# PraKesEy/EEGNetReplication

Hardware: AMD Instinct MI355X
Metric: train trials/sec (fwd+bwd) EEGNet-8,2 22ch x 256 (higher is better)
Workload: dtype fp32; 1 GPU; EEGNet-8,2 train step (fwd+CE+bwd+clamps+Adam), 22ch x 256, batch 4096/GPU, p=0.5, fp32 HIP kernels; model=EEGNet-8,2, global_batch=4096, seq_len=256, channels=22, parallelism=dp1

## Files before the change

eegnetreplication_amd/csrc/eegnet_stream.hip:

```cpp

namespace eeg {

constexpr int NTB = 512;
constexpr int NWB = NTB / 64;
constexpr int RPW = F2MAX / NWB;
constexpr int WGPC = 2;
constexpr int WPEB = NWB * WGPC / 4;

__device__ __forceinline__ int fir_row(int lane) { return (lane >> 3) & 1; }
__device__ __forceinline__ int fir_oct(int lane) { return (lane & 7) | ((lane >> 4) << 3); }
#define EEG_XP(TT, g) (((TT) && ((TT) & 3) == 0) ? (TT) : (g).XP)
#define EEG_NO(TT) ((TT) ? ((TT) + 7) / 8 : ((T + 7) >> 3))
#define EEG_MO(TT) ((TT) ? (((TT) + 7) / 8 + 31) / 32 : 4)

typedef __attribute__((address_space(1))) void gvoid_t;
typedef __attribute__((address_space(3))) void lvoid_t;
__device__ __forceinline__ void x_dma(const float* __restrict__ xb, int C, int T, int RS, int LP, float* Xs,
                                      int wave, int lane) {
    if ((T & 255) == 0) {
        const int np = T >> 8;
        for (int i = wave; i < C * np; i += NWB) {
            const int c = i / np, p = i - c * np;
            __builtin_amdgcn_global_load_lds((gvoid_t*)(xb + (size_t)c * T + 256 * p + 4 * lane),
                                             (lvoid_t*)(Xs + c * RS + LP + 256 * p), 16, 0, 0);
// ... 577 lines not shown
            float a[4];
#pragma unroll
            for (int i = 0; i < 4; ++i) a[i] = (4 * q + i < T) ? w[G_::OFF + i] : 0.f;
            s0 += (a[0] + a[1]) + (a[2] + a[3]);
#pragma unroll
            for (int d = 0; d < K1; ++d) {
                float acc = G0[d];
#pragma unroll
                for (int i = 0; i < 4; ++i) acc = fmaf(a[i], w[G_::OFF + i + d], acc);
                G0[d] = acc;
            }
        }
        float* orow = out + (size_t)b * NV;
#pragma unroll
        for (int i = 0; i < NEI; ++i) {
            if (ea[i] >= 0) {
                const float* xa = Xb + LP + ea[i];
                float acc = 0.f;
                if (eb[i] >= 0) {
                    const float* xb2 = Xb + LP + eb[i];
                    for (int c = 0; c < C; ++c) acc = fmaf(xa[c * RS], xb2[c * RS], acc);
                } else {
                    for (int c = 0; c < C; ++c) acc += xa[c * RS];
                }
                orow[K1 + 1 + tid + NTB * i] = acc;
            }
        }
        constexpr int NR = (K1 + 1 + 3) & ~3, NQ = NR / 4;
        float rv[NR];
#pragma unroll
        for (int d = 0; d < K1; ++d) rv[d] = G0[d];
        rv[K1] = s0;
#pragma unroll
        for (int i = K1 + 1; i < NR; ++i) rv[i] = 0.f;
        wave_reduce<NR>(rv);
        if ((lane & 15) == 0) {
            const int r0 = (lane >> 4) * NQ;
#pragma unroll
            for (int j = 0; j < NQ; ++j)
                if (j + r0 <= K1) red[wave * (K1 + 1) + j + r0] = rv[j];
        }
        __syncthreads();
        if (tid <= K1) {
            float t = 0.f;
            for (int w = 0; w < NWB; ++w) t += red[w * (K1 + 1) + tid];
            orow[tid] = t;
        }
    }
}

template <int K1, int CC, int TT, int FF, bool FOLD>
__device__ __forceinline__ void pass_b_body(const Geo& g, const float* __restrict__ prm,
                                            const float* coef,
                                            const float* __restrict__ vg,
                                            const uint8_t* __restrict__ mask2,
                                            float* __restrict__ d2g, float* __restrict__ E1g,
                                            float* __restrict__ E2g, float* __restrict__ q3g,
                                            float* __restrict__ r3g, float* __restrict__ part,
                                            FinArgs fa, const FoldCall& fc, float* sm) {
    EEG_DIMS_NT(g, NTB);
    TRACE(g, 1, TR_ENTRY);
    unsigned dk0;
    if (FOLD) {
        const eegnet_fold f = fold_rec(fc);
        char* ws = (char*)f.ws;
        prm = f.params;
        coef = (const float*)(ws + fc.off.coef);
        vg = (const float*)(ws + fc.off.v);
        mask2 = nullptr;
        d2g = (float*)(ws + fc.off.d2); E1g = (float*)(ws + fc.off.E1); E2g = (float*)(ws + fc.off.E2);
        q3g = (float*)(ws + fc.off.q3); r3g = (float*)(ws + fc.off.r3);
        part = (float*)(ws + fc.off.partB);
        fa = fold_fin(fc, f, TK_B, 1, 0, true, false, g.nparam);
        dk0 = fold_drop_key(fc, f, 0);
    } else {
        dk0 = drop_key(g, 0);
    }
    float* D2s = sm;
    float* Qs0 = D2s + F2 * RS2;
    float* Wt = Qs0 + 2 * F2 * RS2;
    const int tid = threadIdx.x, lane = tid & 63;
    const int wave = __builtin_amdgcn_readfirstlane(tid >> 6);
    int b0, b1;
    trial_range(g, b0, b1);
    const int NO = EEG_NO(TT);
    constexpr int MO = EEG_MO(TT);
    const int hr = fir_row(lane), oh = RPW * wave + hr;
    constexpr bool VPF = TT != 0;
    float vpf[MO][8];
    if (VPF && b0 < b1) v_load<MO>(vg, b0, F2, NO, oh, lane, vpf);

    for (int i = tid; i < 3 * F2 * RS2; i += NTB) sm[i] = 0.f;
    for (int i = tid; i < F2MAX * (K2 + F2MAX); i += NTB) {
        float v = 0.f;
        if (i < F2MAX * K2) { if (i < F2 * K2) v = prm[g.o_w2 + i]; }
        else {
            const int j = (i - F2MAX * K2) / F2MAX, c = (i - F2MAX * K2) % F2MAX;
            if (j < F2 && c < F2) v = prm[g.o_W3 + j * F2 + c];
        }
        Wt[i] = v;
    }
    float sr[RPW], sr2[RPW];
#pragma unroll
    for (int r = 0; r < RPW; ++r) { sr[r] = 0.f; sr2[r] = 0.f; }
    float alh, beh, gah, bth;
    {
        const int oo = oh < F2 ? oh : 0;
        alh = coef[CF_AL2 * CSTR + oo]; beh = coef[CF_BE2 * CSTR + oo];
        gah = prm[g.o_g2 + oo]; bth = prm[g.o_b2 + oo];
    }
    __syncthreads();

    TRACE(g, 1, TR_PRO);
    TRACE_DECL();
    drain_prologue_loads();
    for (int b = b0; b < b1; ++b) {
        const int bn = b + 1;
        pace_prio(b - b0, b1 - b0);
        float* Qs = Qs0 + ((b - b0) & 1) * F2 * RS2;
        float vc[MO][8];
        if constexpr (VPF) {
#pragma unroll
            for (int m = 0; m < MO; ++m)
#pragma unroll
                for (int i = 0; i < 8; ++i) vc[m][i] = vpf[m][i];
            if (bn < b1) v_load<MO>(vg, bn, F2, NO, oh, lane, vpf);
        } else {
            v_load<MO>(vg, b, F2, NO, oh, lane, vc);
        }
        TRACE_PH(g, 1, 0, tph_);
        float d2v[MO][2], e1v[MO][2], e2v[MO][2];
        if (oh < F2) {
            float* drow = D2s + oh * RS2 + LP2;
#pragma unroll
            for (int m = 0; m < MO; ++m) {
                const int oc = fir_oct(lane) + 32 * m;
                if (oc >= NO) break;
#pragma unroll
                for (int h = 0; h < 2; ++h) {
                    const int q = 2 * oc + h;
                    float pe = 0.f, e1 = 0.f, e2 = 0.f;
#pragma unroll
                    for (int i = 4 * h; i < 4 * h + 4; ++i) {
                        const float xh = fmaf(alh, vc[m][i], beh);
                        const float z = fmaf(gah, xh, bth);
                        const float dz = elu_d(z);
                        pe += z > 0.f ? z : dz - 1.f;
                        e1 += dz;
                        e2 = fmaf(dz, xh, e2);
                    }
                    const float d2 = q < T1 ? pe * 0.25f * keep_mul(g, mask2, dk0, (unsigned)((b * F2 + oh) * T1 + q)) : 0.f;
                    d2v[m][h] = d2; e1v[m][h] = e1; e2v[m][h] = e2;
                    if (q < T1) drow[q] = d2;
                }
            }
        }
        wave_lds_fence();
        TRACE_PH(g, 1, 1, tph_);
#pragma unroll
        for (int r = 0; r < RPW; ++r) {
            const int o = RPW * wave + r;
            if (o < F2) {
                const float* dr = D2s + o * RS2 + LP2 - 7;
                const float* w2 = Wt + o * K2;
                for (int t = lane; t < T1; t += 64) {
                    float a = 0.f;
#pragma unroll
                    for (int k = 0; k < K2; ++k) a = fmaf(w2[k], dr[t + k], a);
                    Qs[o * RS2 + t] = a;
                    q3g[((size_t)b * F2 + o) * T1 + t] = a;
                }
            }
        }
        TRACE_PH(g, 1, 2, tph_);
        if (oh < F2) {
#pragma unroll
            for (int m = 0; m < MO; ++m) {
                const int oc = fir_oct(lane) + 32 * m;
                if (oc >= NO) break;
#pragma unroll
                for (int h = 0; h < 2; ++h) {
                    const int q = 2 * oc + h;
                    if (q < T1) {
                        const size_t gi = ((size_t)b * F2 + oh) * T1 + q;
                        st_pol<EEGNET_NT_MID>(d2v[m][h], d2g + gi); st_pol<EEGNET_NT_MID>(e1v[m][h], E1g + gi);
                        st_pol<EEGNET_NT_MID>(e2v[m][h], E2g + gi);
                    }
                }
            }
        }
        TRACE_PH(g, 1, 3, tph_);
        barrier_lds();
        TRACE_PH(g, 1, 4, tph_);
        for (int t = lane; t < T1; t += 64) {
            float qv[F2MAX];
#pragma unroll
            for (int i = 0; i < F2MAX; ++i) qv[i] = i < F2 ? Qs[i * RS2 + t] : 0.f;
#pragma unroll
            for (int r = 0; r < RPW; ++r) {
                const int o = RPW * wave + r;
                if (o < F2) {
                    const float* w3 = Wt + F2MAX * K2 + o * F2MAX;
                    float rr = 0.f;
#pragma unroll
                    for (int i = 0; i < F2MAX; ++i) rr = fmaf(w3[i], qv[i], rr);
                    r3g[((size_t)b * F2 + o) * T1 + t] = rr;
                    sr[r] += rr;
                    sr2[r] = fmaf(rr, rr, sr2[r]);
                }
            }
        }
        TRACE_PH(g, 1, 5, tph_);
    }
    TRACE_LOOP(g, 1);
    tail_prio();
    {
        float rv[4] = {sr[0], sr[1], sr2[0], sr2[1]};
        wave_reduce<4>(rv);
        const int k = lane >> 4, o = RPW * wave + (k & 1);
        if ((lane & 15) == 0 && o < F2) {
            float* row = part + (size_t)blockIdx.x * g.nB;
            pub(row + ((k < 2 ? 0 : F2) + o), rv[0]);
        }
    }
    {
        double* dsm = (double*)sm;
        if (grid_reduce(g, part, g.nB, fa, dsm)) { fin2(g, dsm + 2, fa); TRACE(g, 1, TR_FIN); }
    }
}

template <int K1, int CC, int TT, int FF, bool FOLD = false>
__global__ __launch_bounds__(NTB, WPEB) void k_pass_b(Geo g, const float* __restrict__ prm,
                                                      const float* coef,
                                                      const float* __restrict__ vg,
                                                      const uint8_t* __restrict__ mask2,
                                                      float* __restrict__ d2g, float* __restrict__ E1g,
                                                      float* __restrict__ E2g, float* __restrict__ q3g,
                                                      float* __restrict__ r3g, float* __restrict__ part,
                                                      FinArgs fa, FoldCall fc) {
    extern __shared__ __attribute__((aligned(16))) float sm[];
    pass_b_body<K1, CC, TT, FF, FOLD>(g, prm, coef, vg, mask2, d2g, E1g, E2g, q3g, r3g, part, fa, fc, sm);
}

#ifndef EEGNET_LDSX_E
#define EEGNET_LDSX_E 0
#endif
template <int K1, int CC, int TT, int FF, bool FOLD>
__device__ __forceinline__ void pass_e_body(const Geo& g, const float* prm,
                                            const float* coef,
                                            const float* __restrict__ x,
                                            const float* __restrict__ sg, const float* __restrict__ vg,
                                            const float* __restrict__ dp2g,
                                            float* __restrict__ part, FinArgs fa, const FoldCall& fc, float* sm) {
    using G_ = KG<K1>;
    EEG_DIMS_NT(g, NTB);
    const int XP = EEG_XP(TT, g);
    TRACE(g, 4, TR_ENTRY);
    const int64_t* perm = nullptr;
    long long row0 = 0;
    if (FOLD) {
        const eegnet_fold f = fold_rec(fc);
        char* ws = (char*)f.ws;
        prm = f.params;
        coef = (const float*)(ws + fc.off.coef);
        x = f.x;
        perm = f.perm; row0 = fc.row0;
        sg = (const float*)(ws + fc.off.s);
        vg = (const float*)(ws + fc.off.v);
        dp2g = (const float*)(ws + fc.off.dp2);
        part = (float*)(ws + fc.off.partE);
        fa = fold_fin(fc, f, TK_E, 0, 0, false, true, g.nparam);
    }
    constexpr int NTS = FF ? 1 : RPW;
    const int D = FF ? 2 : g.D;
    const int QR = FF ? FF / 2 : g.QR;
    float* const Ss = sm;
    float* const Dys = Ss + F2 * RS;
    float* const Xb = Dys + F2 * RS;
    float* const DP = Xb + C * RS;
    float* red = sm;
    const int tid = threadIdx.x, lane = tid & 63;
    const int wave = __builtin_amdgcn_readfirstlane(tid >> 6);
    int b0, b1;
    trial_range(g, b0, b1);
    const int li = lane & 15, lk = lane >> 4;
    constexpr bool XDMA = TT != 0;
    static_assert(!XDMA || (CC && FF), "LDS-DMA staging is specialised to compile-time C and F2");

    TRACE_PS(g, 0);
    if constexpr (!XDMA) zero_fill<false>(sm, (2 * F2 + C) * RS, F2, RS, LP, T, tid);
    TRACE_PS(g, 1);
    float tap[NTS][K1];
    float* CT = DP + ((F2 * T1 + 3) & ~3);
    const int NO = EEG_NO(TT);
    constexpr int MO = EEG_MO(TT);
    const int hr = fir_row(lane), oh = RPW * wave + hr;
    constexpr bool ONEOC = FF && TT && (EEG_NO(TT) <= 32) && (FF == RPW * NWB);
    constexpr bool EINPL = ONEOC || XDMA;
    float* const Eb = EINPL ? Dys : Ss;
    constexpr bool XDMA_ = TT != 0;
    constexpr bool DPDMA_ = XDMA_ && FF && ((FF * (TT / 4)) % 256 == 0);
    constexpr bool PIPEE = ONEOC && XDMA_ && DPDMA_ && (TT / 4 == 64) && (TT == 256);
    float sdyl = 0.f, sdyvl = 0.f;
    constexpr int NWT = (15 + K1 - 1) / 16 + 1;
    floatx4 cq[RPW][NWT];
#pragma unroll
    for (int r = 0; r < RPW; ++r)
#pragma unroll
        for (int j = 0; j < NWT; ++j) cq[r][j] = (floatx4){0.f, 0.f, 0.f, 0.f};
    const int wpc = NWB / NCT;
    const bool gemm_on = wave < wpc * NCT;
    const int ct = gemm_on ? wave / wpc : 0, part_ = gemm_on ? wave - ct * wpc : 0;
    const int kg0 = (NT16 * part_) / wpc, kg1 = gemm_on ? (NT16 * (part_ + 1)) / wpc : 0;
    floatx4 xacc = {0.f, 0.f, 0.f, 0.f};
    constexpr int MS = TT ? (TT + 63) / 64 : 16;
    float pws[XDMA ? 1 : RPW][XDMA ? 1 : MS];
    auto s_rows_load = [&](int bb) {
        if constexpr (!XDMA) {
#pragma unroll
            for (int r = 0; r < RPW; ++r) {
                const float* src = sg + ((size_t)bb * F2 + min(RPW * wave + r, F2 - 1)) * s_pitch(T);
#pragma unroll
                for (int k = 0; k < MS; ++k) pws[r][k] = src[min(lane + 64 * k, T - 1)];
            }
        }
    };
    auto s_rows_put = [&]() {
        if constexpr (!XDMA) {
#pragma unroll
            for (int r = 0; r < RPW; ++r) {
                const int o = RPW * wave + r;
#pragma unroll
                for (int k = 0; k < MS; ++k)
                    if (o < F2 && lane + 64 * k < T) Ss[o * RS + LP + lane + 64 * k] = pws[r][k];
            }
        }
    };
    float pfx[XDMA ? 1 : PF];
    constexpr bool VPF = XDMA;
    float vpf[MO][8];
    constexpr int NDP = (CC && TT) ? (FF * (TT / 4) + NTB - 1) / NTB : 8;
    const int ndp = F2 * T1;
    float pdp[NDP];
    constexpr bool DPDMA = TT && FF && ((FF * (TT / 4)) % 256 == 0);
    if (b0 < b1) {
        if constexpr (XDMA) s_dma_asm(sg + (size_t)b0 * F2 * s_pitch(T), F2, T, RS, LP, Ss, wave, lane);
        else s_rows_load(b0);
        TRACE_PS(g, 3);
        if constexpr (DPDMA) flat_dma_asm(dp2g + (size_t)b0 * ndp, ndp, DP, wave, lane);
        else {
#pragma unroll
            for (int j = 0; j < NDP; ++j) pdp[j] = dp2g[(size_t)b0 * ndp + min(tid + NTB * j, ndp - 1)];
#pragma unroll
            for (int j = 0; j < NDP; ++j)
                if (tid + NTB * j < ndp) DP[tid + NTB * j] = pdp[j];
            for (int i = tid + NTB * NDP; i < ndp; i += NTB) DP[i] = dp2g[(size_t)b0 * ndp + i];
        }
        if constexpr (VPF) v_load<MO>(vg, b0, F2, NO, oh, lane, vpf);
        TRACE_PS(g, 4);
    }
    if constexpr (XDMA) zero_pads(sm, 2 * F2 + C, RS, LP, T, tid);
    load_taps<K1, NTS>(g, prm, D, F2, wave, tap);
    TRACE_PS(g, 2);
    {
        float cv = 0.f;
#pragma unroll
        for (int k = 0; k < 8 * RPW; ++k) {
            const int o = RPW * wave + (k >> 3), f = k & 7;
            if (o < F2 && f < 7) {
                const float* src = f == 0 ? coef + CF_AL2 * CSTR : f == 1 ? coef + CF_BE2 * CSTR
                                 : f == 2 ? prm + g.o_g2 : f == 3 ? prm + g.o_b2 : f == 4 ? coef + CF_AO * CSTR
                                 : f == 5 ? coef + CF_BO * CSTR : coef + CF_CO * CSTR;
                const float v = ldc(src + o);
                cv = lane == k ? v : cv;
            }
        }
        if (lane < 8 * RPW && RPW * wave + (lane >> 3) < F2) CT[8 * RPW * wave + lane] = cv;
    }
    adam_scalars_publish(g, fa);
    const int step0 = adam_step0(g, fa);
    if constexpr (XDMA) barrier_vm<0>();
    else __syncthreads();
    if constexpr (!XDMA) {
        if (b0 < b1) {
            s_rows_put();
            x_prefetch<PF, NTB>(x + fold_row(perm, row0, b0) * (C * XP), C, T, pfx, tid);
            x_store<PF, NTB>(pfx, C, T, RS, LP, Xb, tid);
        }
        __syncthreads();
    }

    TRACE(g, 4, TR_PRO);
    TRACE_DECL();
    drain_prologue_loads();
    for (int b = b0; b < b1; ++b) {
        const int bn = b + 1;
        pace_prio(b - b0, b1 - b0);
        float vc[MO][8];
        if constexpr (VPF) {
#pragma unroll
            for (int m = 0; m < MO; ++m)
#pragma unroll
                for (int i = 0; i < 8; ++i) vc[m][i] = vpf[m][i];
            if constexpr (PIPEE)
                if (bn < b1) v_load<MO>(vg, bn, F2, NO, oh, lane, vpf);
        } else {
            v_load<MO>(vg, b, F2, NO, oh, lane, vc);
        }
        TRACE_PH(g, 4, 0, tph_);
        if (oh < F2) {
            float* drow = Dys + oh * RS + LP;
            const floatx4 c0 = lds_ld4(CT + 8 * oh), c1 = lds_ld4(CT + 8 * oh + 4);
            const float alh = c0[0], beh = c0[1], gah = c0[2], bth = c0[3];
            const float Aoh = c1[0], Boh = c1[1], Coh = c1[2];
#pragma unroll
            for (int m = 0; m < MO; ++m) {
                const int oc = fir_oct(lane) + 32 * m;
                if (oc >= NO) break;
                float dpq[2];
#pragma unroll
                for (int h = 0; h < 2; ++h)
                    dpq[h] = EEGNET_LDSX_E == 1 ? 0.01f * (oc + h) : (2 * oc + h < T1) ? DP[oh * T1 + 2 * oc + h] * 0.25f : 0.f;
                float dy[8];
#pragma unroll
                for (int i = 0; i < 8; ++i) {
                    const bool in = 8 * oc + i < T;
                    const float v = in ? vc[m][i] : 0.f;
                    const float xh = fmaf(alh, v, beh);
                    const float z = fmaf(gah, xh, bth);
                    const float dz = dpq[i >> 2] * elu_d(z);
                    float d = fmaf(Aoh, dz, fmaf(Coh, xh, Boh));
                    d = in ? d : 0.f;
                    dy[i] = d;
                    sdyl += d;
                    sdyvl = fmaf(d, v, sdyvl);
                }
                if (EEGNET_LDSX_E != 5)
                    lds_st_oct(drow + 8 * oc, oc, (floatx4){dy[0], dy[1], dy[2], dy[3]}, (floatx4){dy[4], dy[5], dy[6], dy[7]});
            }
        }
        TRACE_PH(g, 4, 1, tph_);
        wave_lds_fence();
        if constexpr (PIPEE) {
            if (bn < b1) {
#pragma unroll
                for (int r = 0; r < RPW; ++r) {
                    const int o = RPW * wave + r;
                    if (EEGNET_LDSX_E != 7) dma4(dp2g + (size_t)bn * ndp + o * T1 + lane, DP + o * T1);
                }
            }
        }
        if constexpr (XDMA)
            if (EEGNET_LDSX_E != 7) x_dma_asm(x + fold_row(perm, row0, b) * (C * XP), C, T, XP, RS, LP, Xb, wave, lane);
        TRACE_PH(g, 4, 2, tph_);
        {
            float tl[K1];
            half_taps<K1, NTS>(tap, hr, tl);
            if constexpr (ONEOC) {
                constexpr int NT16C = (TT + 15) / 16, KQC = (NT16C + 3) / 4, NQ = RPW * KQC * NWT;
                const int oc = fir_oct(lane);
                float w[4 * G_::NW8];
                if (EEGNET_LDSX_E == 2) {
#pragma unroll
                    for (int i = 0; i < 4 * G_::NW8; ++i) w[i] = 0.001f * (lane + i);
                } else
                    lds_window<G_::NW8>(Dys + oh * RS + 8 * oc, w);
                float e[8];
#pragma unroll
                for (int i = 0; i < 8; ++i) e[i] = 0.f;
#pragma unroll
                for (int m = 0; m < K1; ++m) {
#pragma unroll
                    for (int i = 0; i < 8; ++i) e[i] = fmaf(tl[K1 - 1 - m], w[G_::OFFD + i + m], e[i]);
#pragma unroll
                    for (int n = (m * NQ) / K1; n < ((m + 1) * NQ) / K1; ++n) {
                        const int r = n / (KQC * NWT), ks = (n / NWT) % KQC, j = n % NWT;
                        const int o = RPW * wave + r, a = 4 * ks + lk;
                        const bool on = a < NT16C;
                        const int ac = on ? a : 0;
                        float av = EEGNET_LDSX_E == 3 ? 0.01f * (li + n) : Dys[o * RS + LP + li + 16 * ac];
                        float bv = EEGNET_LDSX_E == 3 ? 0.02f * (lk + n) : Ss[o * RS + G_::OFF + li + 16 * (ac + j)];
                        av = on ? av : 0.f;
                        bv = on ? bv : 0.f;
                        cq[r][j] = __builtin_amdgcn_mfma_f32_16x16x4f32(av, bv, cq[r][j], 0, 0, 0);
                    }
                }
                float* erow = Dys + oh * RS + LP;
#pragma unroll
                for (int i = 0; i < 8; ++i) e[i] = (8 * oc + i < T) ? e[i] : 0.f;
                wave_lds_fence();
                if (EEGNET_LDSX_E != 6)
                    lds_st_oct(erow + 8 * oc, oc, (floatx4){e[0], e[1], e[2], e[3]}, (floatx4){e[4], e[5], e[6], e[7]});
                if constexpr (PIPEE) {
                    if (bn < b1 && EEGNET_LDSX_E != 7) {
#pragma unroll
                        for (int r = 0; r < RPW; ++r) {
                            const int o = RPW * wave + r;
                            dma16(sg + ((size_t)bn * F2 + o) * s_pitch(T) + 4 * lane, Ss + o * RS + LP);
                        }
                    }
                }
            } else {
                const int KQ = (NT16 + 3) >> 2;
#pragma unroll
                for (int r = 0; r < RPW; ++r) {
                    const int o = RPW * wave + r;
                    if (o < F2) {
                        const float* dyr = Dys + o * RS + LP + li;
                        const float* sr = Ss + o * RS + G_::OFF + li;
                        for (int ks = 0; ks < KQ; ++ks) {
                            const int a = 4 * ks + lk;
                            const bool on = a < NT16;
                            const int ac = on ? a : 0;
                            float av = dyr[16 * ac];
                            av = on ? av : 0.f;
#pragma unroll
                            for (int j = 0; j < NWT; ++j) {
                                float bv = sr[16 * (ac + j)];
                                bv = on ? bv : 0.f;
                                cq[r][j] = __builtin_amdgcn_mfma_f32_16x16x4f32(av, bv, cq[r][j], 0, 0, 0);
                            }
                        }
                    }
                }
                if constexpr (EINPL) {
                    float e[MO][8];
                    if (oh < F2) {
                        const float* dyr = Dys + oh * RS;
                        constexpr bool TAIL1 = TT && (TT % 8 == 1) && (EEG_NO(TT) % 32 == 1);
#pragma unroll
                        for (int m = 0; m < MO; ++m) {
                            const int oc = min(fir_oct(lane) + 32 * m, NO - 1);
                            float w[4 * G_::NW8];
                            lds_window<G_::NW8>(dyr + 8 * oc, w);
#pragma unroll
                            for (int i = 0; i < 8; ++i) e[m][i] = 0.f;
                            if (TAIL1 && m == MO - 1) {
#pragma unroll
                                for (int k = 0; k < K1; ++k) e[m][0] = fmaf(tl[K1 - 1 - k], w[G_::OFFD + k], e[m][0]);
                            } else {
#pragma unroll
                                for (int k = 0; k < K1; ++k)
#pragma unroll
                                    for (int i = 0; i < 8; ++i)
                                        e[m][i] = fmaf(tl[K1 - 1 - k], w[G_::OFFD + i + k], e[m][i]);
                            }
                        }
                    }
                    wave_lds_fence();
                    if (oh < F2) {
                        float* erow = Dys + oh * RS + LP;
#pragma unroll
                        for (int m = 0; m < MO; ++m) {
                            const int oc = fir_oct(lane) + 32 * m;
                            if (oc < NO) {
#pragma unroll
                                for (int i = 0; i < 8; ++i) e[m][i] = (8 * oc + i < T) ? e[m][i] : 0.f;
                                lds_st_oct(erow + 8 * oc, oc, (floatx4){e[m][0], e[m][1], e[m][2], e[m][3]},
                                           (floatx4){e[m][4], e[m][5], e[m][6], e[m][7]});
                            }
                        }
                    }
                } else
                if (oh < F2) {
                    const float* dyr = Dys + oh * RS;
                    float* erow = Ss + oh * RS + LP;
                    for (int oc = fir_oct(lane); oc < NO; oc += 32) {
                        float w[4 * G_::NW8];
                        lds_window<G_::NW8>(dyr + 8 * oc, w);
                        float e[8];
#pragma unroll
                        for (int i = 0; i < 8; ++i) e[i] = 0.f;
#pragma unroll
                        for (int k = 0; k < K1; ++k)
#pragma unroll
                            for (int i = 0; i < 8; ++i) e[i] = fmaf(tl[K1 - 1 - k], w[G_::OFFD + i + k], e[i]);
#pragma unroll
                        for (int i = 0; i < 8; ++i) e[i] = (8 * oc + i < T) ? e[i] : 0.f;
                        lds_st_oct(erow + 8 * oc, oc, (floatx4){e[0], e[1], e[2], e[3]}, (floatx4){e[4], e[5], e[6], e[7]});
                    }
                }
            }
        }
        TRACE_PH(g, 4, 3, tph_);
        if (!DPDMA && bn < b1) {
#pragma unroll
            for (int j = 0; j < NDP; ++j) pdp[j] = dp2g[(size_t)bn * ndp + min(tid + NTB * j, ndp - 1)];
        }
        if constexpr (PIPEE) {
            if (bn < b1) barrier_vm<RPW>();
            else barrier_vm<0>();
        } else if constexpr (XDMA) barrier_vm<0>();
        else __syncthreads();
        TRACE_PH(g, 4, 4, tph_);
        if (!PIPEE && bn < b1) {
            if constexpr (XDMA) s_dma_asm(sg + (size_t)bn * F2 * s_pitch(T), F2, T, RS, LP, Ss, wave, lane);
            else {
                s_rows_load(bn);
                x_prefetch<PF, NTB>(x + fold_row(perm, row0, bn) * (C * XP), C, T, pfx, tid);
            }
            if constexpr (DPDMA) flat_dma_asm(dp2g + (size_t)bn * ndp, ndp, DP, wave, lane);
            asm volatile("" ::: "memory");
            if constexpr (VPF) v_load<MO>(vg, bn, F2, NO, oh, lane, vpf);
        }
        TRACE_PH(g, 4, 5, tph_);
        if (gemm_on) {
            const int c = ct * 16 + li;
            const bool aon = li < F2, bon = c < C;
            if constexpr (TT != 0 && TT / 128 >= 2) {
                constexpr int KGP = 8 * (TT / 128);
                const int lo = 64 * (lk & 1) + 4 * (lk >> 1);
                const float* arow = Eb + (aon ? li : 0) * RS + LP + lo;
                const float* brow = Xb + (bon ? c : li) * RS + LP + lo;
                for (int kg = kg0; kg < kg1; ++kg) {
                    const int to = kg < KGP ? 128 * (kg >> 3) + 8 * (kg & 7) : 16 * kg + 4 * lk - lo;
                    floatx4 a4, b4;
                    if (EEGNET_LDSX_E == 4) {
                        a4 = (floatx4){0.01f * kg, 0.02f * li, 0.f, 1.f};
                        b4 = (floatx4){0.03f * kg, 0.01f * lk, 1.f, 0.f};
                    } else {
                        a4 = lds_ld4(arow + to);
                        b4 = lds_ld4(brow + to);
                    }
                    if (!aon) a4 = (floatx4){0.f, 0.f, 0.f, 0.f};
                    if (!bon) b4 = (floatx4){0.f, 0.f, 0.f, 0.f};
#pragma unroll
                    for (int e = 0; e < 4; ++e) xacc = __builtin_amdgcn_mfma_f32_16x16x4f32(a4[e], b4[e], xacc, 0, 0, 0);
                }
            } else {
                const float* arow = Eb + (aon ? li : 0) * RS + LP + 2 * lk;
                const float* brow = Xb + (bon ? c : (li < C ? li : 0)) * RS + LP + 2 * lk;
                const int o8 = 8 + opaque0();
                const float* arow8 = arow + o8;
                const float* brow8 = brow + o8;
                for (int kg = kg0; kg < kg1; ++kg) {
                    floatx2 a0 = lds_ld2(arow + 16 * kg), a1 = lds_ld2(arow8 + 16 * kg);
                    floatx2 b0 = lds_ld2(brow + 16 * kg), b1 = lds_ld2(brow8 + 16 * kg);
                    if (!aon) { a0 = (floatx2){0.f, 0.f}; a1 = a0; }
                    if (!bon) { b0 = (floatx2){0.f, 0.f}; b1 = b0; }
                    xacc = __builtin_amdgcn_mfma_f32_16x16x4f32(a0[0], b0[0], xacc, 0, 0, 0);
                    xacc = __builtin_amdgcn_mfma_f32_16x16x4f32(a0[1], b0[1], xacc, 0, 0, 0);
                    xacc = __builtin_amdgcn_mfma_f32_16x16x4f32(a1[0], b1[0], xacc, 0, 0, 0);
                    xacc = __builtin_amdgcn_mfma_f32_16x16x4f32(a1[1], b1[1], xacc, 0, 0, 0);
                }
            }
        }
        if (bn < b1) {
            if constexpr (!DPDMA) {
#pragma unroll
                for (int j = 0; j < NDP; ++j) {
                    const int i = tid + NTB * j;
                    if (i < ndp) DP[i] = pdp[j];
                }
            }
        }
        TRACE_PH(g, 4, 6, tph_);
        if constexpr (PIPEE) barrier_vm<0>();
        else if constexpr (XDMA && DPDMA && VPF) barrier_vm<2 * MO>();
        else if constexpr (XDMA || DPDMA) barrier_vm<0>();
        else __syncthreads();
        if constexpr (!XDMA)
            if (bn < b1) {
                x_store<PF, NTB>(pfx, C, T, RS, LP, Xb, tid);
                s_rows_put();
            }
        TRACE_PH(g, 4, 7, tph_);
    }
    TRACE_LOOP(g, 4);
    tail_prio();
    __syncthreads();

    float* row = part + (size_t)blockIdx.x * g.nE;
    {
        constexpr int NR = 4, NH = NR / 2;
        float rv[NR];
        rv[0] = sdyl; rv[1] = sdyvl; rv[2] = 0.f; rv[3] = 0.f;
        {
            const int ocl = lane & 31;
            const int src = (ocl & 7) | ((ocl >> 3) << 4) | ((lane >> 5) << 3);
#pragma unroll
            for (int k = 0; k < NR; ++k) rv[k] = __shfl(rv[k], src, 64);
        }
        half_reduce<NR>(rv);
        if ((lane & 15) == 0) {
            const int o = RPW * wave + (lane >> 5), off = ((lane >> 4) & 1) * NH;
            if (o < F2) {
#pragma unroll
                for (int j = 0; j < NH; ++j) {
                    const int idx = j + off;
                    if (idx == 0) pub(row + (QR * K1 + F2 * C + o), rv[j]);
                    else if (idx == 1) pub(row + (QR * K1 + F2 * C + F2 + o), rv[j]);
                }
            }
        }
    }
    {
        float* CQ = red + NWB * 256 + wave * (256 * NWT);
        const bool grp = QR != F2;
        float qg = 0.f;
#pragma unroll
        for (int r = 0; r < RPW; ++r) {
            const int o = RPW * wave + r;
            if (o < F2) {
#pragma unroll
                for (int j = 0; j < NWT; ++j)
#pragma unroll
                    for (int q = 0; q < 4; ++q) CQ[(4 * lk + q) * (16 * NWT) + 16 * j + li] = cq[r][j][q];
                wave_lds_fence();
                if (lane < K1) {
                    float a = 0.f;
#pragma unroll
                    for (int u = 0; u < 16; ++u) a += CQ[u * (16 * NWT) + u + lane];
                    if (grp) qg += a;
                    else pub(row + (o * K1 + lane), a);
                }
                wave_lds_fence();
            }
        }
        if (grp && RPW * wave < F2 && lane < K1) pub(row + (wave * K1 + lane), qg);
    }
#pragma unroll
    for (int q = 0; q < 4; ++q) red[wave * 256 + (4 * lk + q) * 16 + li] = gemm_on ? xacc[q] : 0.f;
    __syncthreads();
    for (int p = tid; p < F2 * C; p += NTB) {
        const int oo2 = p / C, c = p - oo2 * C;
        const int ct2 = c >> 4, cc = c & 15;
        float a = 0.f;
        for (int w = ct2 * wpc; w < (ct2 + 1) * wpc; ++w) a += red[w * 256 + oo2 * 16 + cc];
        pub(row + (QR * K1 + p), a);
    }
    {
        double* dsm = (double*)sm;
        Fin5Stage f5;
        if (!g.defer) fin5_load(g, fa, blockIdx.x, f5);
        if (grid_reduce(g, part, g.nE, fa, dsm)) {
            fin5_body<true>(g, prm, dsm + 2, dsm + tail_s_doubles(g.nE), fa, blockIdx.x, f5);
            TRACE(g, 4, TR_FIN);
        } else {
            adam_slice(g, fa, blockIdx.x, gridDim.x, step0);
        }
    }
}

template <int K1, int CC, int TT, int FF, bool FOLD = false>
__global__ __launch_bounds__(NTB, WPEB) void k_pass_e(Geo g, const float* prm,
                                                      const float* coef,
                                                      const float* __restrict__ x,
                                                      const float* __restrict__ sg, const float* __restrict__ vg,
                                                      const float* __restrict__ dp2g,
                                                      float* __restrict__ part, FinArgs fa, FoldCall fc) {
    extern __shared__ __attribute__((aligned(16))) float sm[];
    pass_e_body<K1, CC, TT, FF, FOLD>(g, prm, coef, x, sg, vg, dp2g, part, fa, fc, sm);
}

}
```

Measured before the change: 19.00 million trials/s.

## Software-pipeline dy2 computation into the GEMM MFMA stream one batch ahead

For the pipelined shape (T=256, one octet per lane), the elementwise dy2 gradient for the next batch is now computed interleaved with the depthwise GEMM MFMAs of the current batch and held in registers until the next iteration stores it to LDS. The DP tile DMA is issued two batches ahead, and the loop barrier waits only on the older loads (vmcnt RPW). The aim is to hide the VALU dy2 work under MFMA latency and to take the DP load off the critical path. In exchange it adds register pressure and extra buffering of the next batch's DP, and the DMA-ahead pattern carries a risk of LDS hazards.

```diff
diff --git a/eegnetreplication_amd/csrc/eegnet_stream.hip b/eegnetreplication_amd/csrc/eegnet_stream.hip
--- a/eegnetreplication_amd/csrc/eegnet_stream.hip
+++ b/eegnetreplication_amd/csrc/eegnet_stream.hip
@@ -903,6 +903,27 @@
     constexpr bool DPDMA_ = XDMA_ && FF && ((FF * (TT / 4)) % 256 == 0);
     constexpr bool PIPEE = ONEOC && XDMA_ && DPDMA_ && (TT / 4 == 64) && (TT == 256);
     float sdyl = 0.f, sdyvl = 0.f;
+    struct Dy2C { float alh, beh, gah, bth, Aoh, Boh, Coh; };
+    auto dy2_consts = [&]() {
+        const floatx4 c0 = lds_ld4(CT + 8 * oh), c1 = lds_ld4(CT + 8 * oh + 4);
+        return Dy2C{c0[0], c0[1], c0[2], c0[3], c1[0], c1[1], c1[2]};
+    };
+    auto dy2_dp = [&](int oc, float (&dpq)[2]) {
+#pragma unroll
+        for (int h = 0; h < 2; ++h)
+            dpq[h] = EEGNET_LDSX_E == 1 ? 0.01f * (oc + h) : (2 * oc + h < T1) ? DP[oh * T1 + 2 * oc + h] * 0.25f : 0.f;
+    };
+    auto dy2_at = [&](const Dy2C& k, float vin, float dq, bool in) {
+        const float v = in ? vin : 0.f;
+        const float xh = fmaf(k.alh, v, k.beh);
+        const float z = fmaf(k.gah, xh, k.bth);
+        const float dz = dq * elu_d(z);
+        float d = fmaf(k.Aoh, dz, fmaf(k.Coh, xh, k.Boh));
+        d = in ? d : 0.f;
+        sdyl += d;
+        sdyvl = fmaf(d, v, sdyvl);
+        return d;
+    };
     constexpr int NWT = (15 + K1 - 1) / 16 + 1;
     floatx4 cq[RPW][NWT];
 #pragma unroll
@@ -994,65 +1015,70 @@
     TRACE(g, 4, TR_PRO);
     TRACE_DECL();
     drain_prologue_loads();
+    float dyh[PIPEE ? 8 : 1];
+    auto dp2_ahead = [&](int bb) {
+        wave_lds_fence();
+#pragma unroll
+        for (int r = 0; r < RPW; ++r) {
+            const int o = RPW * wave + r;
+            if (EEGNET_LDSX_E != 7) dma4(dp2g + (size_t)bb * ndp + o * T1 + lane, DP + o * T1);
+        }
+    };
+    if constexpr (PIPEE) {
+        if (b0 < b1) {
+            const Dy2C k = dy2_consts();
+            float dpq[2];
+            dy2_dp(fir_oct(lane), dpq);
+#pragma unroll
+            for (int i = 0; i < 8; ++i) dyh[i] = dy2_at(k, vpf[0][i], dpq[i >> 2], true);
+            if (b0 + 1 < b1) dp2_ahead(b0 + 1);
+        }
+    }
     for (int b = b0; b < b1; ++b) {
         const int bn = b + 1;
         pace_prio(b - b0, b1 - b0);
-        float vc[MO][8];
-        if constexpr (VPF) {
-#pragma unroll
-            for (int m = 0; m < MO; ++m)
-#pragma unroll
-                for (int i = 0; i < 8; ++i) vc[m][i] = vpf[m][i];
-            if constexpr (PIPEE)
-                if (bn < b1) v_load<MO>(vg, bn, F2, NO, oh, lane, vpf);
+        if constexpr (PIPEE) {
+            const int oc = fir_oct(lane);
+            if (EEGNET_LDSX_E != 5)
+                lds_st_oct(Dys + oh * RS + LP + 8 * oc, oc, (floatx4){dyh[0], dyh[1], dyh[2], dyh[3]},
+                           (floatx4){dyh[4], dyh[5], dyh[6], dyh[7]});
+            if (bn < b1) v_load<MO>(vg, bn, F2, NO, oh, lane, vpf);
+            TRACE_PH(g, 4, 0, tph_);
+            wave_lds_fence();
+            TRACE_PH(g, 4, 1, tph_);
         } else {
-            v_load<MO>(vg, b, F2, NO, oh, lane, vc);
-        }
-        TRACE_PH(g, 4, 0, tph_);
-        if (oh < F2) {
-            float* drow = Dys + oh * RS + LP;
-            const floatx4 c0 = lds_ld4(CT + 8 * oh), c1 = lds_ld4(CT + 8 * oh + 4);
-            const float alh = c0[0], beh = c0[1], gah = c0[2], bth = c0[3];
-            const float Aoh = c1[0], Boh = c1[1], Coh = c1[2];
-#pragma unroll
-            for (int m = 0; m < MO; ++m) {
-                const int oc = fir_oct(lane) + 32 * m;
-                if (oc >= NO) break;
-                float dpq[2];
-#pragma unroll
-                for (int h = 0; h < 2; ++h)
-                    dpq[h] = EEGNET_LDSX_E == 1 ? 0.01f * (oc + h) : (2 * oc + h < T1) ? DP[oh * T1 + 2 * oc + h] * 0.25f : 0.f;
-                float dy[8];
-#pragma unroll
-                for (int i = 0; i < 8; ++i) {
-                    const bool in = 8 * oc + i < T;
-                    const float v = in ? vc[m][i] : 0.f;
-                    const float xh = fmaf(alh, v, beh);
-                    const float z = fmaf(gah, xh, bth);
-                    const float dz = dpq[i >> 2] * elu_d(z);
-                    float d = fmaf(Aoh, dz, fmaf(Coh, xh, Boh));
-                    d = in ? d : 0.f;
-                    dy[i] = d;
-                    sdyl += d;
-                    sdyvl = fmaf(d, v, sdyvl);
-                }
-                if (EEGNET_LDSX_E != 5)
-                    lds_st_oct(drow + 8 * oc, oc, (floatx4){dy[0], dy[1], dy[2], dy[3]}, (floatx4){dy[4], dy[5], dy[6], dy[7]});
-            }
-        }
-        TRACE_PH(g, 4, 1, tph_);
-        wave_lds_fence();
-        if constexpr (PIPEE) {
-            if (bn < b1) {
-#pragma unroll
-                for (int r = 0; r < RPW; ++r) {
-                    const int o = RPW * wave + r;
-                    if (EEGNET_LDSX_E != 7) dma4(dp2g + (size_t)bn * ndp + o * T1 + lane, DP + o * T1);
-                }
-            }
+            float vc[MO][8];
+            if constexpr (VPF) {
+#pragma unroll
+                for (int m = 0; m < MO; ++m)
+#pragma unroll
+                    for (int i = 0; i < 8; ++i) vc[m][i] = vpf[m][i];
+            } else {
+                v_load<MO>(vg, b, F2, NO, oh, lane, vc);
+            }
+            TRACE_PH(g, 4, 0, tph_);
+            if (oh < F2) {
+                float* drow = Dys + oh * RS + LP;
+                const Dy2C k = dy2_consts();
+#pragma unroll
+                for (int m = 0; m < MO; ++m) {
+                    const int oc = fir_oct(lane) + 32 * m;
+                    if (oc >= NO) break;
+                    float dpq[2];
+                    dy2_dp(oc, dpq);
+                    float dy[8];
+#pragma unroll
+                    for (int i = 0; i < 8; ++i) dy[i] = dy2_at(k, vc[m][i], dpq[i >> 2], 8 * oc + i < T);
+                    if (EEGNET_LDSX_E != 5)
+                        lds_st_oct(drow + 8 * oc, oc, (floatx4){dy[0], dy[1], dy[2], dy[3]}, (floatx4){dy[4], dy[5], dy[6], dy[7]});
+                }
+            }
+            TRACE_PH(g, 4, 1, tph_);
+            wave_lds_fence();
         }
         if constexpr (XDMA)
-            if (EEGNET_LDSX_E != 7) x_dma_asm(x + fold_row(perm, row0, b) * (C * XP), C, T, XP, RS, LP, Xb, wave, lane);
+            if (EEGNET_LDSX_E != 7)
+                x_dma_asm(x + fold_row(perm, row0, b) * (C * XP), C, T, XP, RS, LP, Xb, wave, lane);
         TRACE_PH(g, 4, 2, tph_);
         {
             float tl[K1];
@@ -1093,6 +1119,8 @@
                 if (EEGNET_LDSX_E != 6)
                     lds_st_oct(erow + 8 * oc, oc, (floatx4){e[0], e[1], e[2], e[3]}, (floatx4){e[4], e[5], e[6], e[7]});
                 if constexpr (PIPEE) {
+#pragma unroll
+                    for (int i = 0; i < 8; ++i) asm volatile("" : "+v"(vpf[0][i]));
                     if (bn < b1 && EEGNET_LDSX_E != 7) {
 #pragma unroll
                         for (int r = 0; r < RPW; ++r) {
@@ -1213,6 +1241,41 @@
                 const int lo = 64 * (lk & 1) + 4 * (lk >> 1);
                 const float* arow = Eb + (aon ? li : 0) * RS + LP + lo;
                 const float* brow = Xb + (bon ? c : li) * RS + LP + lo;
+                if constexpr (PIPEE) {
+                    constexpr int NCTC = (CC + 15) / 16, WPC = NWB / NCTC, KGW = ((TT + 15) / 16) / WPC;
+                    static_assert(WPC * NCTC == NWB && KGW * WPC == (TT + 15) / 16 && KGW * WPC <= KGP && 8 % KGW == 0 &&
+                                  4 * KGW == 2 * 8, "dws GEMM split of the pipelined shape");
+                    const int to0 = 128 * (kg0 >> 3) + 8 * (kg0 & 7);
+                    auto gemm = [&](auto ahead) {
+                        floatx4 a4[KGW], b4[KGW];
+#pragma unroll
+                        for (int j = 0; j < KGW; ++j) {
+                            if (EEGNET_LDSX_E == 4) {
+                                a4[j] = (floatx4){0.01f * (kg0 + j), 0.02f * li, 0.f, 1.f};
+                                b4[j] = (floatx4){0.03f * (kg0 + j), 0.01f * lk, 1.f, 0.f};
+                            } else {
+                                a4[j] = lds_ld4(arow + to0 + 8 * j);
+                                b4[j] = lds_ld4(brow + to0 + 8 * j);
+                            }
+                            if (!aon) a4[j] = (floatx4){0.f, 0.f, 0.f, 0.f};
+                            if (!bon) b4[j] = (floatx4){0.f, 0.f, 0.f, 0.f};
+                        }
+                        Dy2C k = {};
+                        float dpq[2] = {0.f, 0.f};
+                        if constexpr (decltype(ahead)::value) {
+                            k = dy2_consts();
+                            dy2_dp(fir_oct(lane), dpq);
+                        }
+#pragma unroll
+                        for (int n = 0; n < 4 * KGW; ++n) {
+                            xacc = __builtin_amdgcn_mfma_f32_16x16x4f32(a4[n >> 2][n & 3], b4[n >> 2][n & 3], xacc, 0, 0, 0);
+                            if constexpr (decltype(ahead)::value)
+                                if (n & 1) dyh[n >> 1] = dy2_at(k, vpf[0][n >> 1], dpq[n >> 3], true);
+                        }
+                    };
+                    if (bn < b1) gemm(std::true_type{});
+                    else gemm(std::false_type{});
+                } else
                 for (int kg = kg0; kg < kg1; ++kg) {
                     const int to = kg < KGP ? 128 * (kg >> 3) + 8 * (kg & 7) : 16 * kg + 4 * lk - lo;
                     floatx4 a4, b4;
@@ -1255,8 +1318,13 @@
                 }
             }
         }
+        if constexpr (PIPEE)
+            if (bn + 1 < b1) dp2_ahead(bn + 1);
         TRACE_PH(g, 4, 6, tph_);
-        if constexpr (PIPEE) barrier_vm<0>();
+        if constexpr (PIPEE) {
+            if (bn + 1 < b1) barrier_vm<RPW>();
+            else barrier_vm<0>();
+        }
         else if constexpr (XDMA && DPDMA && VPF) barrier_vm<2 * MO>();
         else if constexpr (XDMA || DPDMA) barrier_vm<0>();
         else __syncthreads();
```

New measurement: 19.24 million trials/s (median of 6 runs). 1.01x the previous value.
